# postworthy/ghost

Measured on AMD Instinct MI355X. Metric: swapped frames/sec at 256×256 bf16, 1/2/4/8 MI355X; AAD decoder HBM GB/s, higher is better.
Workload: dtype bf16; 1 GPU; BASELINE config 2: batch=64 synthetic 256x256 aligned faces per GPU, AEI_Net unet num_blocks=2, faceshifter_batch (u8 in -> u8 out, device-resident; D2H in legs.d2h); global_batch=64, per_gpu_batch=64, backbone=unet, num_blocks=2, identities=1, parallelism=dp1, batches_in_flight=2

## Files before the change

### ghost_amd/csrc/conv_halo.hip

```cpp
#include <cstdlib>
#include <type_traits>
#include <utility>

#include "conv_halo.h"
#include "ghost_common.h"

namespace ghost {

template <int TH_, int TW_, int WM_, int WN_, int IMG_ = 1>
struct HaloCfg {
  static constexpr int TH = TH_, TW = TW_, WM = WM_, WN = WN_, IMG = IMG_;
  static constexpr int BN = 64 * WN, NW = WM * WN, WPI = WM / IMG;
  static constexpr int HWW = TW + 2, HHH = TH + 2;
  static constexpr int HIMG = HHH * HWW;
  static constexpr int HP = IMG * HIMG;
  static constexpr int HPIECES = (HP + 15) / 16;
  static constexpr int WPIECES = 9 * BN / 16;
  static constexpr int HALO_B = HPIECES * 1024;
  static constexpr int LDS_B = HALO_B + 9 * BN * 64;
  static constexpr int HPW = (HPIECES + NW - 1) / NW;
  static constexpr int WPW = (WPIECES + NW - 1) / NW;
  static_assert(IMG * TH * TW == 64 * WM, "each wave owns 64 output pixels");
  static_assert(IMG == 1 || (WN == 1 && WM % IMG == 0), "multi-image tiles: whole waves per image");
  GHOST_DEV static int img(int w) { return IMG > 1 ? w / WPI : 0; }
// ... 334 lines not shown
    r.y0 = ty * G::TH;
    r.x0 = tx * TW;
    r.n0 = nt * 64;
    return r;
  };
  int h_off[HPW];
  unsigned h_ok = 0u;
  long dma_base = 0;
  int dma_n0 = 0;
  auto set_dma_tile = [&](const Tile& t) {
    dma_base = t.base * a.ldx;
    dma_n0 = t.n0;
    h_ok = 0u;
#pragma unroll
    for (int j = 0; j < HPW; ++j) {
      const int piece = wid + j * NW;
      const int P = piece * 16 + prow;
      const int im = IMG > 1 ? P / G::HIMG : 0, hp = P - im * G::HIMG;
      const int hy = hp / HWW, hx = hp - hy * HWW;
      const int iy = t.y0 - 1 + hy, ix = t.x0 - 1 + hx;
      const bool ok = piece < HPIECES && P < HP && iy >= 0 && iy < a.H && ix >= 0 && ix < a.W;
      h_off[j] = ok ? ((im * a.H + iy) * a.W + ix) * a.ldx + ((slot ^ hswz(P)) * 8) : 0;
      h_ok |= (ok ? 1u : 0u) << j;
    }
  };
  auto issue_piece = [&](unsigned char* buf, int cb, auto jt) {
    constexpr int jj = decltype(jt)::value;
#if defined(__HIP_DEVICE_COMPILE__)
    if constexpr (jj < HPW) {
      const int piece = wid + jj * NW;
      if (piece < HPIECES && !(DBG & 2)) {
        const T* __restrict__ xs = ax_ + dma_base + cb * 32;
        const void* src = ((h_ok >> jj) & 1u) ? (const void*)(xs + h_off[jj]) : (const void*)g_halo_zero;
        __builtin_amdgcn_global_load_lds(src, buf + piece * 1024, 16, 0, 0);
      }
    } else if constexpr (!RESW && !(DBG & 4)) {
      constexpr int j = jj - HPW;
      const int piece = wid + j * NW;
      if (piece < WPIECES) {
        const T* __restrict__ ws = aw_ + (long)dma_n0 * a.Kpad + cb * 288;
        __builtin_amdgcn_global_load_lds(ws + w_off[j], buf + HALO_B + piece * 1024, 16, 0, 0);
      }
    }
#endif
  };
  auto issue = [&](unsigned char* buf, int cb) {
#if defined(__HIP_DEVICE_COMPILE__)
    const T* __restrict__ xs = ax_ + dma_base + cb * 32;
#pragma unroll
    for (int j = 0; j < HPW; ++j) {
      const int piece = wid + j * NW;
      if (piece < HPIECES && !(DBG & 2)) {
        const void* src = ((h_ok >> j) & 1u) ? (const void*)(xs + h_off[j]) : (const void*)g_halo_zero;
        __builtin_amdgcn_global_load_lds(src, buf + piece * 1024, 16, 0, 0);
      }
    }
    if constexpr (!RESW && !(DBG & 4)) {
      const T* __restrict__ ws = aw_ + (long)dma_n0 * a.Kpad + cb * 288;
#pragma unroll
      for (int j = 0; j < WPW; ++j) {
        const int piece = wid + j * NW;
        if (piece < WPIECES)
          __builtin_amdgcn_global_load_lds(ws + w_off[j], buf + HALO_B + piece * 1024, 16, 0, 0);
      }
    }
#endif
  };

  f32x4 acc[4][4];
#pragma unroll
  for (int j = 0; j < 4; ++j)
#pragma unroll
    for (int i = 0; i < 4; ++i) acc[j][i] = f32x4{0.f, 0.f, 0.f, 0.f};

  constexpr bool W16 = !EPX && NCB == 2 && IMG == 1 && !(DBG & 16);
  constexpr int LPITCH = 136, LWAVE = 64 * LPITCH;
  constexpr bool LDSW = !EPX && !W16 && IMG == 1 && !RESW && !(DBG & 16) && STAGE_B >= NW * LWAVE;
  const bool plain = !a.scale && !a.shift && a.slope == 1.f && !a.tanh_out;
  constexpr int NST = ((DBG & 48) || EPX) ? 0 : ((W16 || LDSW) ? 8 : 16) + (STATS ? 1 : 0);
  if (nmine == 0) return;
  constexpr bool SPREAD = (DBG & 4096) == 0;
  constexpr int NPIECE = HPW + (RESW ? 0 : WPW);
  constexpr int PPT = 2;
  Tile cur = tile_of(0);
  set_dma_tile(cur);
  issue(lds0, 0);
  __builtin_amdgcn_s_waitcnt(0x0F70);
  int k = 0;
  auto step = [&](const unsigned char* buf, unsigned char* nbuf, auto cbt) {
    constexpr int cb = decltype(cbt)::value;
    if constexpr (cb == 0)
      __builtin_amdgcn_s_waitcnt(((NST >> 4) << 14) | 0x0F70 | (NST & 15));
    else
      __builtin_amdgcn_s_waitcnt(0x0F70);
    __builtin_amdgcn_s_waitcnt(0xC07F);
    __builtin_amdgcn_s_barrier();
    const bool more = cb + 1 < NCB || k + 1 < nmine;
    if constexpr (cb + 1 < NCB) {
      if constexpr (!SPREAD) issue(nbuf, cb + 1);
    } else if (k + 1 < nmine) {
      set_dma_tile(tile_of(k + 1));
      if constexpr (!SPREAD) issue(nbuf, 0);
    }
    constexpr int ncb_next = cb + 1 < NCB ? cb + 1 : 0;
    const unsigned char* wb = RESW ? wres + cb * WBLK_B : buf + HALO_B;
    v8_t<T> wf[2][4], pf[2][4];
    auto load_frags = [&](int tap, v8_t<T> (&w)[4], v8_t<T> (&p)[4]) {
      const int dy = tap / 3, dx = tap - dy * 3;
#pragma unroll
      for (int j = 0; j < 4; ++j) {
        const int n = j * 16 + lr;
        w[j] = *reinterpret_cast<const v8_t<T>*>(wb + (tap * 64 + n) * 64 + ((lq ^ hswz(n)) * 16));
      }
#pragma unroll
      for (int i = 0; i < 4; ++i) {
        const int q = i * 16 + lr;
        const int P = G::himg(wid) + (G::hrow0(wid) + q / TW + dy) * HWW + q % TW + dx;
        p[i] = *reinterpret_cast<const v8_t<T>*>(buf + P * 64 + ((lq ^ hswz(P)) * 16));
      }
    };
    if constexpr ((DBG & 8) == 0) {
      load_frags(0, wf[0], pf[0]);
      if constexpr ((DBG & 64) != 0) load_frags(1, wf[1], pf[1]);
      asm volatile("" ::: "memory");
#pragma unroll
      for (int tap = 0; tap < 9; ++tap) {
        if constexpr ((DBG & 128) == 0) __builtin_amdgcn_s_waitcnt(0xC07F);
        if (tap + 1 < 9 && (DBG & 64) == 0) load_frags(tap + 1, wf[(tap + 1) & 1], pf[(tap + 1) & 1]);
#pragma unroll
        for (int j = 0; j < 4; ++j)
#pragma unroll
          for (int i = 0; i < 4; ++i)
            acc[j][i] = mfma16x16x32<T>(wf[tap & 1][j], pf[tap & 1][i], acc[j][i]);
        if constexpr (SPREAD) {
          if (more) {
            pp_unroll(std::make_integer_sequence<int, 16>{}, [&](auto qt) {
              constexpr int q = decltype(qt)::value;
              const int pc = tap * PPT + q;
              if ((q < PPT || (tap == 8 && pc < NPIECE)) && pc < NPIECE) {
                switch (pc) {
#define GHOST_SPREAD_CASE(N) case N: if constexpr (N < NPIECE) issue_piece(nbuf, ncb_next, std::integral_constant<int, N>{}); break;
                  GHOST_SPREAD_CASE(0) GHOST_SPREAD_CASE(1) GHOST_SPREAD_CASE(2) GHOST_SPREAD_CASE(3)
                  GHOST_SPREAD_CASE(4) GHOST_SPREAD_CASE(5) GHOST_SPREAD_CASE(6) GHOST_SPREAD_CASE(7)
                  GHOST_SPREAD_CASE(8) GHOST_SPREAD_CASE(9) GHOST_SPREAD_CASE(10) GHOST_SPREAD_CASE(11)
                  GHOST_SPREAD_CASE(12) GHOST_SPREAD_CASE(13) GHOST_SPREAD_CASE(14) GHOST_SPREAD_CASE(15)
#undef GHOST_SPREAD_CASE
                  default: break;
                }
              }
            });
          }
        }
        if constexpr ((DBG & 128) == 0) {
          if (tap + 1 < 9 && (DBG & 64) == 0) {
            __builtin_amdgcn_sched_group_barrier(0x100, 8, 0);
            __builtin_amdgcn_sched_group_barrier(0x008, 16, 0);
          } else {
            __builtin_amdgcn_sched_group_barrier(0x008, 16, 0);
          }
          __builtin_amdgcn_sched_barrier(0);
        } else {
          asm volatile("" ::: "memory");
        }
      }
    }
    if constexpr (cb + 1 < NCB) return;
// ... 545 lines not shown
```

### ghost_amd/csrc/conv_igemm.hip

```cpp
#include <cstdio>
#include <cstdlib>

#include "conv_igemm.h"
#include "conv_first.h"
#include "conv_halo.h"
#include "conv_s2.h"
#include "ghost_common.h"

namespace ghost {

struct ConvArgs {
  const void* x;
  const void* w;
  void* y;
  const float* scale;
  const float* shift;
  const void* res;
  const float* prelu;
  void* y2;
  const float* scale2;
  const float* shift2;
  const void* hin;
  const float* stat;
  const float* idgb;
  const float* mask;
  float* partial;
  uint8_t* u8;
  long wpar_stride;
  int B, Hi, Wi, Cin, ldx;
  int Ho, Wo, M;
  int N, Kpad, K, NT;
  int nNt;
  int ldy, ldres, ldh, id_ld, C_aad, ldy2, res_first;
  int stride, ntx, ntaps, tbase, tsign;
  int deconv;
  int nsplit, kt_per_split;
  float slope;
  int tanh_out;
  int nmajor;
  unsigned* sem;
  int fuse;
};

template <typename TO>
GHOST_DEV float epi_std(const ConvArgs& a, float v, int n, long opix) {
  if (a.scale) v *= a.scale[n];
  if (a.shift) v += a.shift[n];
  const float r = a.res ? to_f(reinterpret_cast<const TO*>(a.res)[opix * a.ldres + n]) : 0.f;
  if (a.res_first) v += r;
  const float sl = a.prelu ? a.prelu[n] : a.slope;
  v = v > 0.f ? v : v * sl;
  if (!a.res_first) v += r;
  if (a.tanh_out) v = tanhf(v);
  return v;
}

template <typename TO>
GHOST_DEV void store_std(const ConvArgs& a, float v, int n, long opix) {
  reinterpret_cast<TO*>(a.y)[opix * a.ldy + n] = from_f<TO>(v);
  if (a.y2) reinterpret_cast<TO*>(a.y2)[opix * a.ldy2 + n] = from_f<TO>(v * a.scale2[n] + a.shift2[n]);
  if (a.u8) {
    float t = (v * 0.5f + 0.5f) * 255.0f;
    a.u8[opix * 3 + (2 - n)] = (uint8_t)(int)t;
  }
}

template <typename TO>
GHOST_DEV float epi_aad(const ConvArgs& a, float ga, float ba, int c, long m) {
  const int HW = a.Ho * a.Wo;
  const int b = (int)(m / HW);
  const float hin = to_f(reinterpret_cast<const TO*>(a.hin)[m * a.ldh + c]);
  const float mu = a.stat[((long)b * a.C_aad + c) * 2 + 0];
  const float rs = a.stat[((long)b * a.C_aad + c) * 2 + 1];
  const float h = (hin - mu) * rs;
  const float gi = a.idgb[(long)b * a.id_ld + c];
  const float bi = a.idgb[(long)b * a.id_ld + a.C_aad + c];
  const float Mk = a.mask[m];
  const float A = ga * h + ba;
  const float I = gi * h + bi;
  float out = (1.0f - Mk) * A + Mk * I;
  return out > 0.f ? out : out * a.slope;
}

GHOST_DEV long out_pixel(const ConvArgs& a, long m, int py, int px) {
  if (!a.deconv) return m;
  const int HW = a.Ho * a.Wo;
  const int b = (int)(m / HW);
  const int r = (int)(m - (long)b * HW);
  const int qy = r / a.Wo, qx = r - qy * a.Wo;
  return ((long)b * (2 * a.Ho) + 2 * qy + py) * (2 * a.Wo) + 2 * qx + px;
}

template <typename TO, int BM, int BN, int NTHR>
GHOST_DEV void split_fixup(const ConvArgs& a, int tid, int tile_id, int m0, int n0, int par, float* stage) {
  if (!last_arrival(a.sem + tile_id, (unsigned)a.nsplit, reinterpret_cast<int*>(stage))) return;
  __syncthreads();
  const int py = par >> 1, px = par & 1;
  const int mrows = min(BM, a.M - m0);
  const long sstride = (long)a.M * a.NT;
  const float* pbase = a.partial + (long)par * a.nsplit * sstride + (long)m0 * a.NT + n0;
  const int per_split = mrows * BN, total = a.nsplit * per_split;
  constexpr int U = 8;
  for (int f0 = tid; f0 < total; f0 += U * NTHR) {
    float v[U];
#pragma unroll
    for (int u = 0; u < U; ++u) {
      const int f = min(f0 + u * NTHR, total - 1);
      const int sp = f / per_split, e = f - sp * per_split;
      const int r = e / BN, q = e - r * BN;
      v[u] = ld_dev(pbase + sp * sstride + (long)r * a.NT + q);
    }
#pragma unroll
    for (int u = 0; u < U; ++u)
      if (f0 + u * NTHR < total) stage[f0 + u * NTHR] = v[u];
  }
  __syncthreads();
  if (a.fuse == 1) {
    const int ncol = min(BN, a.N - n0);
    for (int i = tid; i < mrows * ncol; i += NTHR) {
      const int r = i / ncol, q = i - r * ncol;
      float v = 0.f;
      for (int sp = 0; sp < a.nsplit; ++sp) v += stage[sp * per_split + r * BN + q];
      const long op = out_pixel(a, m0 + r, py, px);
      store_std<TO>(a, epi_std<TO>(a, v, n0 + q, op), n0 + q, op);
// ... 273 lines not shown
  const int ncols = (EPI == KEPI_AAD) ? a.C_aad : a.N;
  const int nq = ncols >> 2;
  const long idx = (long)blockIdx.x * 256 + threadIdx.x;
  if (idx >= (long)a.M * nq) return;
  const long m = idx / nq;
  const int c = (int)(idx - m * nq) * 4;
  const float* base = a.partial + ((long)par * a.nsplit * a.M + m) * a.NT;
  const long sstride = (long)a.M * a.NT;
  if constexpr (EPI == KEPI_STD) {
    f32x4 v = f32x4{0.f, 0.f, 0.f, 0.f};
#pragma unroll 8
    for (int s = 0; s < a.nsplit; ++s) v += *reinterpret_cast<const f32x4*>(base + s * sstride + c);
    const long op = out_pixel(a, m, py, px);
#pragma unroll
    for (int e = 0; e < 4; ++e) store_std<TO>(a, epi_std<TO>(a, v[e], c + e, op), c + e, op);
  } else {
    const int ng = (c >> 4) * 32 + (c & 15);
    f32x4 ga = f32x4{0.f, 0.f, 0.f, 0.f}, ba = f32x4{0.f, 0.f, 0.f, 0.f};
#pragma unroll 8
    for (int s = 0; s < a.nsplit; ++s) {
      ga += *reinterpret_cast<const f32x4*>(base + s * sstride + ng);
      ba += *reinterpret_cast<const f32x4*>(base + s * sstride + ng + 16);
    }
#pragma unroll
    for (int e = 0; e < 4; ++e)
      reinterpret_cast<TO*>(a.y)[m * a.ldy + c + e] =
          from_f<TO>(epi_aad<TO>(a, ga[e] + a.shift[ng + e], ba[e] + a.shift[ng + 16 + e], c + e, m));
  }
}

template <typename TO, int EPI>
void launch_reduce(const ConvArgs& a, int ncols, int npar, hipStream_t s) {
  static const int vec = GHOST_KNOB("GHOST_SPLITK_VEC", 1);
  const long total = (long)a.M * ncols;
  if (vec && ncols % 4 == 0 && a.NT % 4 == 0) {
    dim3 grid((unsigned)((total / 4 + 255) / 256), 1, npar);
    hipLaunchKernelGGL((splitk_reduce4_kernel<TO, EPI>), grid, dim3(256), 0, s, a);
  } else {
    dim3 grid((unsigned)((total + 255) / 256), 1, npar);
    hipLaunchKernelGGL((splitk_reduce_kernel<TO, EPI>), grid, dim3(256), 0, s, a);
  }
}

__device__ __attribute__((aligned(16))) unsigned int g_zero_line[64] = {0};

GHOST_DEV int swz(int r, int c) { return c ^ ((r >> 1) & 3); }

template <int N>
GHOST_DEV void wait_vmcnt() {
  asm volatile("s_waitcnt vmcnt(%0)" ::"n"(N) : "memory");
}

template <int LPS, int K>
GHOST_DEV void wait_stages(int after) {
  if constexpr (K <= 0) {
    wait_vmcnt<0>();
  } else {
    if (after >= K) wait_vmcnt<K * LPS>();
    else wait_stages<LPS, K - 1>(after);
  }
}

template <typename T, int BM, int NA, int NB>
GHOST_DEV void glds_issue(const ConvArgs& a, const T* __restrict__ x, const T* const (&b_src)[NB],
                          const long (&a_off)[NA], const uint64_t (&a_mask)[NA], const int (&a_gc)[NA], int wid,
                          int kt, unsigned char* sb) {
#if defined(__HIP_DEVICE_COMPILE__)
  const int k0 = kt * 32;
  const int cb = kt / a.ntaps, tap = kt - cb * a.ntaps;
  const int ty = tap / a.ntx, tx = tap - ty * a.ntx;
  const long toff = ((long)a.tsign * ty * a.Wi + a.tsign * tx) * a.ldx + cb * 32;
#pragma unroll
  for (int j = 0; j < NA; ++j) {
    const void* src = ((a_mask[j] >> tap) & 1ull) ? (const void*)(x + a_off[j] + toff + a_gc[j])
                                                 : (const void*)g_zero_line;
    __builtin_amdgcn_global_load_lds(src, sb + (wid * NA + j) * 1024, 16, 0, 0);
  }
#pragma unroll
  for (int j = 0; j < NB; ++j)
    __builtin_amdgcn_global_load_lds(b_src[j] + k0, sb + BM * 64 + (wid * NB + j) * 1024, 16, 0, 0);
#endif
}

template <typename T, int BM, int BN, int STAGES, int EPI, int WSL = 0>
__global__ void __launch_bounds__(WSL ? 512 : 256) conv_glds_kernel(const ConvArgs a) {
  typedef T TI;
  typedef T TO;
  constexpr int WM = WaveGrid<BM, BN>::WM, WN = WaveGrid<BM, BN>::WN;
  constexpr int WTM = BM / WM, WTN = BN / WN;
  constexpr int TM = WTM / 16, TN = WTN / 16;
  constexpr int NA = BM / 64, NB = BN / 64;
  constexpr int LPS = NA + NB;
  constexpr int STAGE_B = (BM + BN) * 64;
  static_assert(BM % 64 == 0 && BN % 64 == 0, "v2 tile");
  static_assert(EPI != KEPI_AAD || (TN % 2 == 0 && WTN % 32 == 0), "AAD epilogue needs gamma/beta tile pairs");
  static_assert((STAGES - 2) * LPS <= 63, "vmcnt range");
  __shared__ __attribute__((aligned(1024))) unsigned char lds[STAGES * STAGE_B];

  const int tid = threadIdx.x, wid = __builtin_amdgcn_readfirstlane(tid >> 6), lane = tid & 63, lr = lane & 15,
            lq = lane >> 4;
  const bool loads = !WSL || wid >= 4, computes = !WSL || wid < 4;
  const int lw = WSL ? wid - 4 : wid;
  const int tile = xcd_remap(blockIdx.x, gridDim.x);
  const int nMt = gridDim.x / a.nNt;
  const int nt = a.nmajor ? tile / nMt : tile % a.nNt, mt = a.nmajor ? tile % nMt : tile / a.nNt;
  const int m0 = mt * BM, n0 = nt * BN;
  const int split = blockIdx.y, par = blockIdx.z, py = par >> 1, px = par & 1;
  const TI* __restrict__ x = reinterpret_cast<const TI*>(a.x);
  const TI* __restrict__ w = reinterpret_cast<const TI*>(a.w) + par * a.wpar_stride;
  const int nk = a.Kpad / 32;
  const int kt0 = split * a.kt_per_split;
  const int kt1 = min(nk, kt0 + a.kt_per_split);

  const int lrow = lane >> 2, pc = lane & 3;
  const int HoWo = a.Ho * a.Wo;
  const int tby = a.deconv ? py : a.tbase, tbx = a.deconv ? px : a.tbase;
  const int nty = a.K / (a.Cin * a.ntx);
  long a_off[NA];
  uint64_t a_mask[NA];
  int a_gc[NA];
#pragma unroll
  for (int j = 0; j < NA; ++j) {
    const int r = 16 * (lw * NA + j) + lrow;
    const int m = m0 + r;
    a_gc[j] = swz(r, pc) * 8;
    a_off[j] = 0;
    a_mask[j] = 0ull;
    if (m < a.M) {
      const int b = m / HoWo;
      const int rr = m - b * HoWo;
      const int oy = rr / a.Wo, ox = rr - oy * a.Wo;
      const int iyb = oy * a.stride + tby, ixb = ox * a.stride + tbx;
      a_off[j] = ((long)(b * a.Hi + iyb) * a.Wi + ixb) * a.ldx;
      uint64_t mk = 0ull;
      for (int ty = 0; ty < nty; ++ty) {
        const int iy = iyb + a.tsign * ty;
        if (iy < 0 || iy >= a.Hi) continue;
        for (int tx = 0; tx < a.ntx; ++tx) {
          const int ix = ixb + a.tsign * tx;
          if (ix >= 0 && ix < a.Wi) mk |= 1ull << (ty * a.ntx + tx);
        }
      }
      a_mask[j] = mk;
    }
  }
  const TI* b_src[NB];
#pragma unroll
  for (int j = 0; j < NB; ++j) {
    const int r = 16 * (lw * NB + j) + lrow;
    b_src[j] = w + (long)(n0 + r) * a.Kpad + swz(r, pc) * 8;
  }

  const int wm = (wid & 3) / WN, wn = (wid & 3) % WN;
  f32x4 acc[TM][TN];
#pragma unroll
  for (int i = 0; i < TM; ++i)
#pragma unroll
    for (int j = 0; j < TN; ++j) acc[i][j] = f32x4{0.f, 0.f, 0.f, 0.f};

  const int n = kt1 - kt0;
  if (loads) {
#pragma unroll
    for (int s = 0; s < STAGES - 1; ++s)
      if (s < n) glds_issue<T, BM, NA, NB>(a, x, b_src, a_off, a_mask, a_gc, lw, kt0 + s, lds + s * STAGE_B);
  }
  for (int it = 0; it < n; ++it) {
    if (loads) wait_stages<LPS, STAGES - 2>(min(STAGES - 2, n - 1 - it));
    __builtin_amdgcn_s_barrier();
    asm volatile("" ::: "memory");
    if (loads && it + STAGES - 1 < n)
      glds_issue<T, BM, NA, NB>(a, x, b_src, a_off, a_mask, a_gc, lw, kt0 + it + STAGES - 1,
                             lds + ((it + STAGES - 1) % STAGES) * STAGE_B);
    if (!computes) continue;
    const unsigned char* sb = lds + (it % STAGES) * STAGE_B;
    const unsigned char* As = sb;
    const unsigned char* Bs = sb + BM * 64;
    v8_t<T> af[TM], bfv[TN];
#pragma unroll
    for (int i = 0; i < TM; ++i) {
      const int r = wm * WTM + i * 16 + lr;
      af[i] = *reinterpret_cast<const v8_t<T>*>(As + r * 64 + swz(r, lq) * 16);
    }
#pragma unroll
    for (int j = 0; j < TN; ++j) {
      const int r = wn * WTN + j * 16 + lr;
      bfv[j] = *reinterpret_cast<const v8_t<T>*>(Bs + r * 64 + swz(r, lq) * 16);
    }
#pragma unroll
    for (int i = 0; i < TM; ++i)
#pragma unroll
      for (int j = 0; j < TN; ++j) acc[i][j] = mfma16x16x32<T>(af[i], bfv[j], acc[i][j]);
  }

  if constexpr (EPI == KEPI_SPLIT) {
    if (computes) {
#pragma unroll
      for (int i = 0; i < TM; ++i) {
#pragma unroll
        for (int r = 0; r < 4; ++r) {
          const int m = m0 + wm * WTM + i * 16 + lq * 4 + r;
          if (m >= a.M) continue;
          float* dst = a.partial + (((long)par * a.nsplit + split) * a.M + m) * a.NT;
#pragma unroll
          for (int j = 0; j < TN; ++j) {
            if (a.sem) st_dev(dst + n0 + wn * WTN + j * 16 + lr, acc[i][j][r]);
            else dst[n0 + wn * WTN + j * 16 + lr] = acc[i][j][r];
          }
        }
      }
    }
    if (a.sem)
      split_fixup<TO, BM, BN, WSL ? 512 : 256>(a, tid, par * gridDim.x + tile, m0, n0, par, reinterpret_cast<float*>(lds));
    return;
  }
  if (!computes) return;
#pragma unroll
  for (int i = 0; i < TM; ++i) {
#pragma unroll
    for (int r = 0; r < 4; ++r) {
      const int m = m0 + wm * WTM + i * 16 + lq * 4 + r;
      if (m >= a.M) continue;
      if constexpr (EPI == KEPI_STD) {
        const long op = out_pixel(a, m, py, px);
#pragma unroll
        for (int j = 0; j < TN; ++j) {
          const int nn = n0 + wn * WTN + j * 16 + lr;
          if (nn < a.N) store_std<TO>(a, epi_std<TO>(a, acc[i][j][r], nn, op), nn, op);
        }
      } else {
#pragma unroll
        for (int jp = 0; jp < TN / 2; ++jp) {
          const int ng = n0 + wn * WTN + (2 * jp) * 16 + lr;
          const int c = (ng >> 5) * 16 + lr;
          if (c < a.C_aad) {
            const float ga = acc[i][2 * jp][r] + a.shift[ng];
            const float ba = acc[i][2 * jp + 1][r] + a.shift[ng + 16];
            reinterpret_cast<TO*>(a.y)[(long)m * a.ldy + c] = from_f<TO>(epi_aad<TO>(a, ga, ba, c, m));
          }
        }
      }
    }
  }
}

namespace {

struct Plan {
  int BM, BN, BK, nNt, nMt, npar, nsplit, kt_per_split, NT, M, Ho, Wo;
  bool fast;
  bool partial;
  int stages;
};


Plan make_plan(const ConvDesc& d) {
  static const int force_bk = GHOST_KNOB("GHOST_CONV_BK", 0);
  Plan p{};
  p.npar = d.kind == CONV_T4S2 ? 4 : 1;
  if (d.kind == CONV_T4S2) {
    p.Ho = d.Hi;
    p.Wo = d.Wi;
  } else {
    p.Ho = (d.Hi + 2 * d.pad - d.kh) / d.stride + 1;
    p.Wo = (d.Wi + 2 * d.pad - d.kw) / d.stride + 1;
  }
  p.M = d.B * p.Ho * p.Wo;
  const bool bf = is16(d.ti);
  const int vec = bf ? 8 : 4;
  p.fast = (d.Cin % 32 == 0) && (d.ldx % vec == 0) && ((uintptr_t)d.x % 16 == 0);
  const bool bk64_ok = bf && p.fast && d.Cin % 64 == 0 && d.Kpad % 64 == 0;
  p.BK = (bk64_ok && d.Kpad >= 4096) ? 64 : 32;
  if (force_bk == 32 || (force_bk == 64 && bk64_ok)) p.BK = force_bk;
  if (!p.fast) {
    p.BN = d.N <= 32 ? 32 : 64;
    p.BM = d.N <= 32 ? 256 : 64;
  } else if (d.epi == EPI_AAD) {
    p.BN = 128;
    p.BM = ((p.M + 127) / 128) * ((d.N + 127) / 128) * p.npar >= 512 ? 128 : 64;
  } else if (d.N <= 16) {
    p.BN = 16; p.BM = 256;
  } else if (d.N <= 32) {
    p.BN = 32; p.BM = 256;
  } else if (d.N <= 64) {
    p.BN = 64; p.BM = (bf && d.kh == 4 && d.stride == 2 && d.kind == CONV_FWD) ? 128 : 256;
  } else {
    p.BN = 128;
    p.BM = ((p.M + 127) / 128) * ((d.N + 127) / 128) * p.npar >= 512 ? 128 : 64;
  }
  if (!p.fast || p.BM >= 256) p.BK = force_bk == 64 && bk64_ok ? 64 : 32;
  static const int deep = GHOST_KNOB("GHOST_CONV_DEEP", 8);
  const long tiles128 = (long)((p.M + 127) / 128) * ((d.N + 127) / 128) * p.npar;
  const bool deep_k = p.M <= 16384 && d.Kpad >= 4096 && tiles128 < 512;
  if (deep > 0 && bf && p.fast && d.to == d.ti && d.N >= 256 && d.Kpad >= 1024 && d.N % 128 == 0 &&
      ((p.M <= 8192 && tiles128 < 256) || deep_k)) {
    p.BM = 128; p.BN = 128; p.BK = 32; p.stages = deep;
  }
#ifdef GHOST_TUNING
  static const char* force_tile = getenv("GHOST_CONV_TILE");
  if (force_tile && p.fast && d.epi != EPI_AAD) {
    int bm = 0, bn = 0;
    if (sscanf(force_tile, "%dx%d", &bm, &bn) == 2 && bn >= d.N / 2 && bm > 0) { p.BM = bm; p.BN = bn; }
  }
#endif
  p.nNt = (d.N + p.BN - 1) / p.BN;
  p.nMt = (p.M + p.BM - 1) / p.BM;
  p.NT = p.nNt * p.BN;
  const int nk = d.Kpad / p.BK;
  const int tiles = p.nMt * p.nNt * p.npar;
  int s = 1;
  if (d.force_split > 0) {
    s = d.force_split;
  } else if (p.stages > 0) {
    static const int deep_target = GHOST_KNOB("GHOST_SPLIT_DEEP", 256);
    static const int deep_minks = GHOST_KNOB("GHOST_SPLIT_DEEP_MINK", 8);
    if (tiles < 256 && nk >= 16) {
      s = (deep_target + tiles - 1) / tiles;
      s = s < nk / deep_minks ? s : nk / deep_minks;
      if (s < 1) s = 1;
    }
  } else if ((tiles < (d.min_wgs > 0 ? d.min_wgs : 256) && nk >= 16) ||
             (d.min_wgs <= 0 && tiles == 256 && nk >= 64)) {
    static const int split_mul = GHOST_KNOB("GHOST_SPLIT_MUL", 2);
    const int target = split_mul * (d.min_wgs > 0 ? d.min_wgs : 256);
    s = (target + tiles - 1) / tiles;
    s = s < nk / 8 ? s : nk / 8;
    if (s < 1) s = 1;
  }
  if (s > nk) s = nk;
  p.kt_per_split = (nk + s - 1) / s;
  p.nsplit = (nk + p.kt_per_split - 1) / p.kt_per_split;
  p.partial = p.nsplit > 1 || (is16(d.ti) && d.to == GHOST_F32);
  return p;
}

ConvArgs make_args(const ConvDesc& d, const Plan& p, float* partial) {
  ConvArgs a{};
  a.x = d.x; a.w = d.w; a.y = d.y;
  a.scale = d.scale; a.shift = d.shift; a.res = d.res;
  a.prelu = d.prelu; a.y2 = d.y2; a.scale2 = d.scale2; a.shift2 = d.shift2; a.ldy2 = d.ldy2;
  a.res_first = d.res_first;
  a.hin = d.hin; a.stat = d.stat; a.idgb = d.idgb; a.mask = d.mask;
  a.partial = partial; a.u8 = d.u8;
  a.wpar_stride = (long)d.Npad * d.Kpad;
  a.B = d.B; a.Hi = d.Hi; a.Wi = d.Wi; a.Cin = d.Cin; a.ldx = d.ldx;
  a.Ho = p.Ho; a.Wo = p.Wo; a.M = p.M;
  a.N = d.N; a.Kpad = d.Kpad; a.NT = p.NT; a.nNt = p.nNt;
  a.ldy = d.ldy; a.ldres = d.ldres; a.ldh = d.ldh; a.id_ld = d.id_ld; a.C_aad = d.C_aad;
  if (d.kind == CONV_T4S2) {
    a.K = 4 * d.Cin; a.stride = 1; a.ntx = 2; a.ntaps = 4; a.tbase = 0; a.tsign = -1; a.deconv = 1;
  } else {
    a.K = d.kh * d.kw * d.Cin; a.stride = d.stride; a.ntx = d.kw; a.ntaps = d.kh * d.kw; a.tbase = -d.pad;
    a.tsign = 1; a.deconv = 0;
  }
  a.nsplit = p.nsplit; a.kt_per_split = p.kt_per_split;
  a.slope = d.slope; a.tanh_out = d.tanh_out;
  a.nmajor = p.stages > 0 ? GHOST_KNOB("GHOST_CONV_NMAJOR", 1) : 0;
  return a;
}

template <typename TI, typename TO, int BM, int BN, int BK, int EPI, bool FAST>
void launch_gemm(const ConvArgs& a, const Plan& p, hipStream_t s) {
  dim3 grid(p.nMt * p.nNt, p.nsplit, p.npar);
  hipLaunchKernelGGL((conv_igemm_kernel<TI, TO, BM, BN, BK, EPI, FAST>), grid, dim3(256), 0, s, a);
}

template <typename TI, typename TO, int EPI, bool FAST>
int dispatch_tile(const ConvArgs& a, const Plan& p, hipStream_t s) {
  const int key = p.BM * 100000 + p.BN * 100 + p.BK;
#define GHOST_TILE(bm, bn, bk) \
  case bm * 100000 + bn * 100 + bk: launch_gemm<TI, TO, bm, bn, bk, EPI, FAST>(a, p, s); return 0;
  if constexpr (!FAST) {
    if constexpr (EPI != KEPI_AAD) {
      switch (key) { GHOST_TILE(256, 32, 32) GHOST_TILE(64, 64, 32) default: break; }
    }
    return -1;
  } else if constexpr (sizeof(TI) == 2) {
    if constexpr (EPI == KEPI_AAD) {
      switch (key) { GHOST_TILE(128, 128, 32) GHOST_TILE(128, 128, 64) GHOST_TILE(64, 128, 32)
                     GHOST_TILE(64, 128, 64) default: break; }
    } else {
      switch (key) { GHOST_TILE(128, 128, 32) GHOST_TILE(128, 128, 64) GHOST_TILE(64, 128, 32)
                     GHOST_TILE(64, 128, 64) GHOST_TILE(256, 64, 32) GHOST_TILE(256, 64, 64)
                     GHOST_TILE(256, 32, 32) GHOST_TILE(256, 32, 64) GHOST_TILE(256, 16, 32)
                     GHOST_TILE(256, 16, 64) GHOST_TILE(128, 64, 32) GHOST_TILE(128, 64, 64)
                     GHOST_TILE(64, 64, 32) GHOST_TILE(64, 64, 64) GHOST_TILE(128, 32, 32)
                     GHOST_TILE(128, 16, 32) default: break; }
    }
    return -1;
  } else {
    if constexpr (EPI == KEPI_AAD) {
      switch (key) { GHOST_TILE(128, 128, 32) GHOST_TILE(64, 128, 32) default: break; }
    } else {
      switch (key) { GHOST_TILE(128, 128, 32) GHOST_TILE(64, 128, 32) GHOST_TILE(256, 64, 32)
                     GHOST_TILE(256, 32, 32) GHOST_TILE(256, 16, 32) default: break; }
    }
    return -1;
  }
#undef GHOST_TILE
}

template <typename T, int EPI>
bool launch_glds(const ConvArgs& a, const Plan& p, hipStream_t s) {
  static const int stages_knob = GHOST_KNOB("GHOST_CONV_STAGES", 3);
  static const int ws = GHOST_KNOB("GHOST_CONV_WS", 1);
  const int stages = p.stages > 0 ? p.stages : stages_knob;
  dim3 grid(p.nMt * p.nNt, p.nsplit, p.npar);
  if constexpr (EPI == KEPI_AAD) {
    if (p.BM == 128 && p.BN == 128 && stages == 8) {
      if (ws)
        hipLaunchKernelGGL((conv_glds_kernel<T, 128, 128, 8, EPI, 4>), grid, dim3(512), 0, s, a);
      else
        hipLaunchKernelGGL((conv_glds_kernel<T, 128, 128, 8, EPI>), grid, dim3(256), 0, s, a);
      return true;
    }
    if (p.BM == 128 && p.BN == 128 && stages == 3 && ws) {
      hipLaunchKernelGGL((conv_glds_kernel<T, 128, 128, 3, EPI, 4>), grid, dim3(512), 0, s, a);
      return true;
    }
    return false;
  }
#define GHOST_G(bm, bn, st)                                                                      \
  if (p.BM == bm && p.BN == bn && stages == st) {                                                \
    if (ws)                                                                                       \
      hipLaunchKernelGGL((conv_glds_kernel<T, bm, bn, st, EPI, 4>), grid, dim3(512), 0, s, a);      \
    else                                                                                          \
      hipLaunchKernelGGL((conv_glds_kernel<T, bm, bn, st, EPI>), grid, dim3(256), 0, s, a);         \
    return true;                                                                                  \
  }
  GHOST_G(128, 128, 8) GHOST_G(128, 128, 6)
  GHOST_G(128, 128, 4) GHOST_G(256, 64, 4) GHOST_G(128, 64, 4) GHOST_G(64, 128, 4)
  GHOST_G(128, 128, 3) GHOST_G(256, 64, 3) GHOST_G(128, 64, 3) GHOST_G(64, 128, 3)
#undef GHOST_G
  return false;
}

template <typename TI, typename TO>
int dispatch_types(const ConvDesc& d, const ConvArgs& a, const Plan& p, hipStream_t s) {
  int rc;
  if constexpr (sizeof(TI) == 2 && sizeof(TO) == 4) {
    if (!p.partial || d.epi != EPI_STD) return -1;
    rc = p.fast ? dispatch_tile<TI, TI, KEPI_SPLIT, true>(a, p, s) : dispatch_tile<TI, TI, KEPI_SPLIT, false>(a, p, s);
    if (rc) return rc;
    const long total = (long)p.M * d.N;
    dim3 grid((unsigned)((total + 255) / 256), 1, p.npar);
    hipLaunchKernelGGL((splitk_reduce_kernel<float, KEPI_STD>), grid, dim3(256), 0, s, a);
    return 0;
  } else {
  static const int use_v2 = GHOST_KNOB("GHOST_CONV_V2", 1);
  if constexpr (sizeof(TI) == 2 && sizeof(TO) == 2) {
    static const int aad_glds = GHOST_KNOB("GHOST_CONV_AAD_GLDS", 0);
    if (use_v2 && p.fast && p.BK == 32 && (d.epi != EPI_AAD || p.stages > 0 || aad_glds) && p.BM <= 128 &&
        p.partial == (p.nsplit > 1)) {
      const bool ok = p.nsplit > 1 ? launch_glds<TI, KEPI_SPLIT>(a, p, s)
                                   : (d.epi == EPI_AAD ? launch_glds<TI, KEPI_AAD>(a, p, s) : launch_glds<TI, KEPI_STD>(a, p, s));
      if (ok) {
        if (p.nsplit > 1 && !a.sem) {
          if (d.epi == EPI_AAD) launch_reduce<TO, KEPI_AAD>(a, d.C_aad, p.npar, s);
          else launch_reduce<TO, KEPI_STD>(a, d.N, p.npar, s);
        }
        return 0;
      }
    }
  }
  if (p.partial) {
    rc = p.fast ? dispatch_tile<TI, TO, KEPI_SPLIT, true>(a, p, s) : dispatch_tile<TI, TO, KEPI_SPLIT, false>(a, p, s);
    if (rc || a.sem) return rc;
    if (d.epi == EPI_AAD) launch_reduce<TO, KEPI_AAD>(a, d.C_aad, p.npar, s);
    else launch_reduce<TO, KEPI_STD>(a, d.N, p.npar, s);
    return 0;
  }
  if (d.epi == EPI_AAD) {
    if (!p.fast) return -1;
    return dispatch_tile<TI, TO, KEPI_AAD, true>(a, p, s);
  }
  return p.fast ? dispatch_tile<TI, TO, KEPI_STD, true>(a, p, s) : dispatch_tile<TI, TO, KEPI_STD, false>(a, p, s);
  }
}

}

size_t conv_workspace_bytes(const ConvDesc& d) {
  if (conv3x3_halo_supported(d) || convT_halo_supported(d) || conv_stem3x3_supported(d) ||
      conv4x4s2_patch_supported(d))
    return 0;
  if (conv_first_supported(d)) return conv_first_workspace_bytes();
  Plan p = make_plan(d);
  if (!p.partial) return 0;
  return (size_t)p.npar * p.nsplit * p.M * p.NT * sizeof(float);
}

int conv_launch(const ConvDesc& d, void* ws, size_t ws_bytes, hipStream_t stream) {
  if (!d.x || !d.w || !d.y || d.B <= 0 || d.Cin <= 0 || d.N <= 0) return -1;
  if (d.Kpad % 32 != 0 || d.Npad < d.N) return -1;
  if (d.y2 && (!d.scale2 || !d.shift2 || d.epi != EPI_STD)) return -1;
  if (d.kind == CONV_FWD && (d.kh * d.kw > 64 || d.kh < 1 || d.kw < 1 || d.stride < 1)) return -1;
  if (d.epi == EPI_AAD && (d.C_aad % 16 != 0 || d.N != 2 * d.C_aad || !d.hin || !d.stat || !d.idgb || !d.mask || !d.shift))
    return -1;
#ifdef GHOST_TUNING
  static const int trace = GHOST_KNOB("GHOST_CONV_TRACE", 0);
  if (trace)
    fprintf(stderr, "[conv] kind=%d B=%d %dx%d Cin=%d N=%d k=%dx%d s=%d halo=%d\n", (int)d.kind, d.B, d.Hi, d.Wi, d.Cin,
            d.N, d.kh, d.kw, d.stride, (int)conv3x3_halo_supported(d));
#endif
  if (conv3x3_halo_supported(d)) return conv3x3_halo(d, stream);
  if (conv_first_supported(d)) return conv_first(d, ws, ws_bytes, stream);
  if (conv_stem3x3_supported(d)) return conv_stem3x3(d, stream);
  if (convT_halo_supported(d)) return convT_halo(d, stream);
  if (conv4x4s2_patch_supported(d) || conv3x3s2_patch_supported(d)) return conv_s2_patch(d, stream);
  Plan p = make_plan(d);
  if (p.NT > d.Npad) return -1;
  const int K = d.kind == CONV_T4S2 ? 4 * d.Cin : d.kh * d.kw * d.Cin;
  if (d.Kpad < K) return -1;
  float* partial = nullptr;
  if (p.partial) {
    size_t need = (size_t)p.npar * p.nsplit * p.M * p.NT * sizeof(float);
    if (!ws || ws_bytes < need) return -1;
    partial = reinterpret_cast<float*>(ws);
  }
  ConvArgs a = make_args(d, p, partial);
  static const int fuse_knob = GHOST_KNOB("GHOST_SPLIT_FUSE", 1);
  static const long fuse_max = (long)GHOST_KNOB("GHOST_SPLIT_FUSE_KB", 32) << 10;
  if (p.partial && p.nsplit > 1 && d.sem && fuse_knob && !(is16(d.ti) && d.to == GHOST_F32) &&
      (long)p.nMt * p.nNt * p.npar <= d.nsem) {
    const long tile_bytes = (long)p.nsplit * (p.M < p.BM ? p.M : p.BM) * p.BN * 4;
    const int vec = is16(d.ti) ? 8 : 4, esz = is16(d.ti) ? 2 : 4;
    static const int stages_knob = GHOST_KNOB("GHOST_CONV_STAGES", 3);
    const long ring = (long)(p.stages > 0 ? p.stages : stages_knob) * (p.BM + p.BN) * 64;
    const long bufs = 2L * (p.BM + p.BN) * (p.BK + vec) * esz;
    static const int use_v2 = GHOST_KNOB("GHOST_CONV_V2", 1);
    const bool deep_glds = use_v2 && (p.stages == 8 || p.stages == 6 || p.stages == 4);
    const long lds = deep_glds ? ring : (ring < bufs ? ring : bufs);
    if (tile_bytes <= lds && (fuse_knob == 2 || tile_bytes <= fuse_max)) {
      a.sem = d.sem;
      a.fuse = d.epi == EPI_AAD ? 2 : 1;
    }
  }
  int rc;
  if (d.ti == GHOST_F32 && d.to == GHOST_F32) rc = dispatch_types<float, float>(d, a, p, stream);
  else if (d.ti == GHOST_BF16 && d.to == GHOST_BF16) rc = dispatch_types<bf16, bf16>(d, a, p, stream);
  else if (d.ti == GHOST_F32 && d.to == GHOST_BF16) rc = dispatch_types<float, bf16>(d, a, p, stream);
  else if (d.ti == GHOST_F16 && d.to == GHOST_F16) rc = dispatch_types<_Float16, _Float16>(d, a, p, stream);
  else if (d.ti == GHOST_F32 && d.to == GHOST_F16) rc = dispatch_types<float, _Float16>(d, a, p, stream);
  else if (d.ti == GHOST_BF16 && d.to == GHOST_F32 && !d.res && !d.y2) rc = dispatch_types<bf16, float>(d, a, p, stream);
  else return -1;
  if (rc) return rc;
  return (int)hipGetLastError();
}

}
```

Before: 11950 frames/s.

## Add 64-deep K-step warp-specialized GEMM ring for deep-stage convolutions

Adds a new conv_glds64_kernel that moves two 32-wide K slices per ring stage (128-byte rows with a new swizzle) using 4 DMA waves and 4 compute waves, with 4 stages and an optional fragment prefetch of the next stage's first half. It is selected by default whenever the plan uses a deep ring and channel/K alignment allows it, replacing the 8-stage 32-deep path. The epilogue is factored into a shared glds_finish helper. The aim is to halve the barrier and wait overhead per K and overlap LDS fragment reads with MFMAs, at the cost of a different LDS budget and a new tuning-only timestamp probe.

```diff
diff --git a/ghost_amd/csrc/conv_halo.hip b/ghost_amd/csrc/conv_halo.hip
--- a/ghost_amd/csrc/conv_halo.hip
+++ b/ghost_amd/csrc/conv_halo.hip
@@ -440,6 +440,7 @@
   constexpr bool SPREAD = (DBG & 4096) == 0;
   constexpr int NPIECE = HPW + (RESW ? 0 : WPW);
   constexpr int PPT = 2;
+  static_assert(NPIECE <= 16, "the spread issue below dispatches pieces 0..15 only");
   Tile cur = tile_of(0);
   set_dma_tile(cur);
   issue(lds0, 0);
diff --git a/ghost_amd/csrc/conv_igemm.hip b/ghost_amd/csrc/conv_igemm.hip
--- a/ghost_amd/csrc/conv_igemm.hip
+++ b/ghost_amd/csrc/conv_igemm.hip
@@ -40,6 +40,9 @@
   int nmajor;
   unsigned* sem;
   int fuse;
+#ifdef GHOST_TUNING
+  int stamps;
+#endif
 };
 
 template <typename TO>
@@ -479,10 +482,13 @@
 #endif
 }
 
+template <typename T, int BM, int BN, int EPI, int NTHR>
+GHOST_DEV void glds_finish(const ConvArgs& a, const f32x4 (&acc)[BM / WaveGrid<BM, BN>::WM / 16][BN / WaveGrid<BM, BN>::WN / 16],
+                           bool computes, int tile, int m0, int n0, unsigned char* lds);
+
 template <typename T, int BM, int BN, int STAGES, int EPI, int WSL = 0>
 __global__ void __launch_bounds__(WSL ? 512 : 256) conv_glds_kernel(const ConvArgs a) {
   typedef T TI;
-  typedef T TO;
   constexpr int WM = WaveGrid<BM, BN>::WM, WN = WaveGrid<BM, BN>::WN;
   constexpr int WTM = BM / WM, WTN = BN / WN;
   constexpr int TM = WTM / 16, TN = WTN / 16;
@@ -588,7 +594,19 @@
 #pragma unroll
       for (int j = 0; j < TN; ++j) acc[i][j] = mfma16x16x32<T>(af[i], bfv[j], acc[i][j]);
   }
-
+  glds_finish<T, BM, BN, EPI, WSL ? 512 : 256>(a, acc, computes, tile, m0, n0, lds);
+}
+
+template <typename T, int BM, int BN, int EPI, int NTHR>
+GHOST_DEV void glds_finish(const ConvArgs& a, const f32x4 (&acc)[BM / WaveGrid<BM, BN>::WM / 16][BN / WaveGrid<BM, BN>::WN / 16],
+                           bool computes, int tile, int m0, int n0, unsigned char* lds) {
+  typedef T TO;
+  constexpr int WM = WaveGrid<BM, BN>::WM, WN = WaveGrid<BM, BN>::WN;
+  constexpr int WTM = BM / WM, WTN = BN / WN;
+  constexpr int TM = WTM / 16, TN = WTN / 16;
+  const int tid = threadIdx.x, wid = tid >> 6, lane = tid & 63, lr = lane & 15, lq = lane >> 4;
+  const int wm = (wid & 3) / WN, wn = (wid & 3) % WN;
+  const int split = blockIdx.y, par = blockIdx.z, py = par >> 1, px = par & 1;
   if constexpr (EPI == KEPI_SPLIT) {
     if (computes) {
 #pragma unroll
@@ -607,7 +625,7 @@
       }
     }
     if (a.sem)
-      split_fixup<TO, BM, BN, WSL ? 512 : 256>(a, tid, par * gridDim.x + tile, m0, n0, par, reinterpret_cast<float*>(lds));
+      split_fixup<TO, BM, BN, NTHR>(a, tid, par * gridDim.x + tile, m0, n0, par, reinterpret_cast<float*>(lds));
     return;
   }
   if (!computes) return;
@@ -640,6 +658,201 @@
   }
 }
 
+GHOST_DEV int swz128(int r, int c) { return c ^ ((r >> 1) & 7); }
+
+constexpr int G64_STAGES = 4, G64_PIECES = 4;
+
+#ifdef GHOST_TUNING
+__device__ unsigned long long g_ring_stamps[16];
+GHOST_DEV unsigned long long ring_stamp() {
+  unsigned long long t;
+  __builtin_amdgcn_sched_barrier(0);
+  asm volatile("s_memtime %0\n\ts_waitcnt lgkmcnt(0)" : "=s"(t)::"memory");
+  __builtin_amdgcn_sched_barrier(0);
+  return t;
+}
+#define GHOST_RING_STAMP(i)                 \
+  if (stamp) {                              \
+    const unsigned long long t_ = ring_stamp(); \
+    seg[i] += t_ - tprev;                   \
+    tprev = t_;                             \
+  }
+#else
+#define GHOST_RING_STAMP(i)
+#endif
+
+template <typename T>
+GHOST_DEV void glds64_issue(const ConvArgs& a, const T* __restrict__ x, const T* const (&b_src)[G64_PIECES],
+                            const long (&a_off)[G64_PIECES], const uint64_t (&a_mask)[G64_PIECES],
+                            const int (&a_gc)[G64_PIECES], const int (&a_half)[G64_PIECES], int lw, int kt,
+                            unsigned char* sb) {
+#if defined(__HIP_DEVICE_COMPILE__)
+  int tap[2];
+  long toff[2];
+#pragma unroll
+  for (int h = 0; h < 2; ++h) {
+    const int cb = (kt + h) / a.ntaps;
+    tap[h] = (kt + h) - cb * a.ntaps;
+    const int ty = tap[h] / a.ntx, tx = tap[h] - ty * a.ntx;
+    toff[h] = ((long)a.tsign * ty * a.Wi + a.tsign * tx) * a.ldx + cb * 32;
+  }
+#pragma unroll
+  for (int j = 0; j < G64_PIECES; ++j) {
+    const int tp = a_half[j] ? tap[1] : tap[0];
+    const long to = a_half[j] ? toff[1] : toff[0];
+    const void* src = ((a_mask[j] >> tp) & 1ull) ? (const void*)(x + a_off[j] + to + a_gc[j])
+                                                 : (const void*)g_zero_line;
+    __builtin_amdgcn_global_load_lds(src, sb + (lw * G64_PIECES + j) * 1024, 16, 0, 0);
+  }
+#pragma unroll
+  for (int j = 0; j < G64_PIECES; ++j)
+    __builtin_amdgcn_global_load_lds(b_src[j] + (long)kt * 32, sb + 128 * 128 + (lw * G64_PIECES + j) * 1024, 16, 0, 0);
+#endif
+}
+
+template <typename T, int EPI, bool PF>
+__global__ void __launch_bounds__(512) conv_glds64_kernel(const ConvArgs a) {
+  constexpr int BM = 128, BN = 128, STAGES = G64_STAGES, NP = G64_PIECES;
+  constexpr int WN = WaveGrid<BM, BN>::WN;
+  constexpr int TM = 4, TN = 4;
+  constexpr int LPS = 2 * NP;
+  constexpr int STAGE_B = (BM + BN) * 128;
+  constexpr int AHEAD = PF ? STAGES - 3 : STAGES - 2;
+  static_assert(BM / 8 == 4 * NP && BN / 8 == 4 * NP, "four DMA waves cover the tile in 8-row pieces");
+  static_assert(STAGES >= 4 && (STAGES - 2) * LPS <= 63, "vmcnt range");
+  __shared__ __attribute__((aligned(1024))) unsigned char lds[STAGES * STAGE_B];
+
+  const int tid = threadIdx.x, wid = __builtin_amdgcn_readfirstlane(tid >> 6), lane = tid & 63, lr = lane & 15,
+            lq = lane >> 4;
+  const bool loads = wid >= 4, computes = wid < 4;
+  const int lw = wid & 3;
+  const int tile = xcd_remap(blockIdx.x, gridDim.x);
+  const int nMt = gridDim.x / a.nNt;
+  const int nt = a.nmajor ? tile / nMt : tile % a.nNt, mt = a.nmajor ? tile % nMt : tile / a.nNt;
+  const int m0 = mt * BM, n0 = nt * BN;
+  const int split = blockIdx.y, par = blockIdx.z, py = par >> 1, px = par & 1;
+  const T* __restrict__ x = reinterpret_cast<const T*>(a.x);
+  const T* __restrict__ w = reinterpret_cast<const T*>(a.w) + par * a.wpar_stride;
+  const int nk = a.Kpad / 32;
+  const int kt0 = split * a.kt_per_split;
+  const int kt1 = min(nk, kt0 + a.kt_per_split);
+  const int n = (kt1 - kt0) >> 1;
+
+  const int lrow = lane >> 3, pc = lane & 7;
+  const int HoWo = a.Ho * a.Wo;
+  const int tby = a.deconv ? py : a.tbase, tbx = a.deconv ? px : a.tbase;
+  const int nty = a.K / (a.Cin * a.ntx);
+  long a_off[NP];
+  uint64_t a_mask[NP];
+  int a_gc[NP], a_half[NP];
+  const T* b_src[NP];
+#pragma unroll
+  for (int j = 0; j < NP; ++j) {
+    const int r = 8 * (lw * NP + j) + lrow;
+    const int c = swz128(r, pc);
+    const int m = m0 + r;
+    a_half[j] = c >> 2;
+    a_gc[j] = (c & 3) * 8;
+    a_off[j] = 0;
+    a_mask[j] = 0ull;
+    if (m < a.M) {
+      const int b = m / HoWo;
+      const int rr = m - b * HoWo;
+      const int oy = rr / a.Wo, ox = rr - oy * a.Wo;
+      const int iyb = oy * a.stride + tby, ixb = ox * a.stride + tbx;
+      a_off[j] = ((long)(b * a.Hi + iyb) * a.Wi + ixb) * a.ldx;
+      uint64_t mk = 0ull;
+      for (int ty = 0; ty < nty; ++ty) {
+        const int iy = iyb + a.tsign * ty;
+        if (iy < 0 || iy >= a.Hi) continue;
+        for (int tx = 0; tx < a.ntx; ++tx) {
+          const int ix = ixb + a.tsign * tx;
+          if (ix >= 0 && ix < a.Wi) mk |= 1ull << (ty * a.ntx + tx);
+        }
+      }
+      a_mask[j] = mk;
+    }
+    b_src[j] = w + (long)(n0 + r) * a.Kpad + c * 8;
+  }
+
+  const int wm = wid / WN, wn = wid % WN;
+  f32x4 acc[TM][TN];
+#pragma unroll
+  for (int i = 0; i < TM; ++i)
+#pragma unroll
+    for (int j = 0; j < TN; ++j) acc[i][j] = f32x4{0.f, 0.f, 0.f, 0.f};
+
+  const int fsw = (lr >> 1) & 7;
+  const unsigned char* fa = lds + (wm * 64 + lr) * 128;
+  const unsigned char* fb = lds + BM * 128 + (wn * 64 + lr) * 128;
+  const int fo[2] = {(lq ^ fsw) * 16, ((4 + lq) ^ fsw) * 16};
+  auto read_half = [&](int slot, int h, v8_t<T> (&af)[TM], v8_t<T> (&bfv)[TN]) {
+#pragma unroll
+    for (int i = 0; i < TM; ++i) af[i] = *reinterpret_cast<const v8_t<T>*>(fa + slot * STAGE_B + i * 2048 + fo[h]);
+#pragma unroll
+    for (int j = 0; j < TN; ++j) bfv[j] = *reinterpret_cast<const v8_t<T>*>(fb + slot * STAGE_B + j * 2048 + fo[h]);
+  };
+  auto mfmas = [&](const v8_t<T> (&af)[TM], const v8_t<T> (&bfv)[TN]) {
+#pragma unroll
+    for (int i = 0; i < TM; ++i)
+#pragma unroll
+      for (int j = 0; j < TN; ++j) acc[i][j] = mfma16x16x32<T>(af[i], bfv[j], acc[i][j]);
+  };
+
+  if (loads) {
+#pragma unroll
+    for (int s = 0; s < STAGES - 1; ++s)
+      if (s < n) glds64_issue<T>(a, x, b_src, a_off, a_mask, a_gc, a_half, lw, kt0 + 2 * s, lds + s * STAGE_B);
+  }
+  v8_t<T> af0[TM], bf0[TN], af1[TM], bf1[TN];
+  if constexpr (PF) {
+    if (loads) wait_stages<LPS, STAGES - 2>(min(STAGES - 2, n - 1));
+    __builtin_amdgcn_s_barrier();
+    asm volatile("" ::: "memory");
+    if (computes && n > 0) read_half(0, 0, af0, bf0);
+  }
+#ifdef GHOST_TUNING
+  const bool stamp = a.stamps && (blockIdx.x | blockIdx.y | blockIdx.z) == 0 && (wid & 3) == 0;
+  unsigned long long seg[4] = {0ull, 0ull, 0ull, 0ull}, tprev = stamp ? ring_stamp() : 0ull;
+#endif
+  for (int it = 0; it < n; ++it) {
+    if (loads) wait_stages<LPS, AHEAD>(min(AHEAD, max(0, n - 1 - (PF ? 1 : 0) - it)));
+    GHOST_RING_STAMP(0)
+    __builtin_amdgcn_s_barrier();
+    asm volatile("" ::: "memory");
+    GHOST_RING_STAMP(1)
+    if (loads && it + STAGES - 1 < n)
+      glds64_issue<T>(a, x, b_src, a_off, a_mask, a_gc, a_half, lw, kt0 + 2 * (it + STAGES - 1),
+                      lds + ((it + STAGES - 1) % STAGES) * STAGE_B);
+    if (!computes) {
+      GHOST_RING_STAMP(3)
+      continue;
+    }
+    const int slot = it % STAGES;
+    if constexpr (PF) {
+      __builtin_amdgcn_s_waitcnt(0xC07F);
+      __builtin_amdgcn_sched_barrier(0);
+      GHOST_RING_STAMP(2)
+    } else {
+      read_half(slot, 0, af0, bf0);
+    }
+    read_half(slot, 1, af1, bf1);
+    mfmas(af0, bf0);
+    if constexpr (PF)
+      if (it + 1 < n) read_half((it + 1) % STAGES, 0, af0, bf0);
+    mfmas(af1, bf1);
+    GHOST_RING_STAMP(3)
+  }
+#ifdef GHOST_TUNING
+  if (stamp && lane == 0) {
+    unsigned long long* o = g_ring_stamps + (wid ? 8 : 0);
+    for (int i = 0; i < 4; ++i) o[i] = seg[i];
+    o[4] = (unsigned long long)n;
+  }
+#endif
+  glds_finish<T, BM, BN, EPI, 512>(a, acc, computes, tile, m0, n0, lds);
+}
+
 namespace {
 
 struct Plan {
@@ -647,7 +860,12 @@
   bool fast;
   bool partial;
   int stages;
+  bool ring64;
 };
+
+long deep_ring_bytes(const Plan& p) {
+  return p.ring64 ? (long)G64_STAGES * (p.BM + p.BN) * 128 : (long)p.stages * (p.BM + p.BN) * 64;
+}
 
 
 Plan make_plan(const ConvDesc& d) {
@@ -726,6 +944,9 @@
   if (s > nk) s = nk;
   p.kt_per_split = (nk + s - 1) / s;
   p.nsplit = (nk + p.kt_per_split - 1) / p.kt_per_split;
+  static const int deep64 = GHOST_KNOB("GHOST_CONV_DEEP64", 1);
+  const int K = (d.kind == CONV_T4S2 ? 4 : d.kh * d.kw) * d.Cin;
+  p.ring64 = deep64 && p.stages > 0 && d.Cin % 64 == 0 && d.Kpad % 64 == 0 && d.Kpad == K && p.kt_per_split % 2 == 0;
   p.partial = p.nsplit > 1 || (is16(d.ti) && d.to == GHOST_F32);
   return p;
 }
@@ -802,6 +1023,33 @@
   static const int ws = GHOST_KNOB("GHOST_CONV_WS", 1);
   const int stages = p.stages > 0 ? p.stages : stages_knob;
   dim3 grid(p.nMt * p.nNt, p.nsplit, p.npar);
+  if (p.ring64) {
+#ifdef GHOST_TUNING
+    static const int pf = GHOST_KNOB("GHOST_CONV_DEEP64_PF", 1);
+    static const int stamps = GHOST_KNOB("GHOST_CONV_STAMPS", 0);
+    ConvArgs b = a;
+    b.stamps = stamps;
+    if (pf) hipLaunchKernelGGL((conv_glds64_kernel<T, EPI, true>), grid, dim3(512), 0, s, b);
+    else hipLaunchKernelGGL((conv_glds64_kernel<T, EPI, false>), grid, dim3(512), 0, s, b);
+    if (stamps) {
+      unsigned long long h[16] = {0};
+      if (hipStreamSynchronize(s) == hipSuccess &&
+          hipMemcpyFromSymbol(h, HIP_SYMBOL(g_ring_stamps), sizeof(h)) == hipSuccess && h[4] > 0 && h[12] > 0) {
+        const double nc = (double)h[4], nd = (double)h[12];
+        fprintf(stderr,
+                "[ring64] M=%d N=%d Kpad=%d nsplit=%d pf=%d steps=%d | compute wave: top->wait %.0f  ->barrier exit %.0f"
+                "  ->fragments back %.0f  ->last MFMA issued %.0f | DMA wave: vmcnt wait %.0f  ->barrier exit %.0f"
+                "  ->next stage issued %.0f  (cycles per 64-deep step)\n",
+                a.M, a.N, a.Kpad, a.nsplit, pf, (int)h[4], h[0] / nc, h[1] / nc, h[2] / nc, h[3] / nc, h[8] / nd,
+                h[9] / nd, h[11] / nd);
+      }
+    }
+    return true;
+#else
+    hipLaunchKernelGGL((conv_glds64_kernel<T, EPI, true>), grid, dim3(512), 0, s, a);
+    return true;
+#endif
+  }
   if constexpr (EPI == KEPI_AAD) {
     if (p.BM == 128 && p.BN == 128 && stages == 8) {
       if (ws)
@@ -922,7 +1170,7 @@
     const long tile_bytes = (long)p.nsplit * (p.M < p.BM ? p.M : p.BM) * p.BN * 4;
     const int vec = is16(d.ti) ? 8 : 4, esz = is16(d.ti) ? 2 : 4;
     static const int stages_knob = GHOST_KNOB("GHOST_CONV_STAGES", 3);
-    const long ring = (long)(p.stages > 0 ? p.stages : stages_knob) * (p.BM + p.BN) * 64;
+    const long ring = p.stages > 0 ? deep_ring_bytes(p) : (long)stages_knob * (p.BM + p.BN) * 64;
     const long bufs = 2L * (p.BM + p.BN) * (p.BK + vec) * esz;
     static const int use_v2 = GHOST_KNOB("GHOST_CONV_V2", 1);
     const bool deep_glds = use_v2 && (p.stages == 8 || p.stages == 6 || p.stages == 4);
```

Measured after the change: 11960 frames/s (median of 2 runs). About the same (+0.1%).
